# JunweiLiang/FVTA_MemexQA

Hardware: AMD Instinct MI355X
Metric: QA-pairs/sec (fwd+bwd) at B=64, 40 photos x 5 streams x 30 tok, h=512 (higher is better)
Workload: dtype bf16; 1 GPU; BASELINE.json configs[2] train step (fwd+bwd+adam), shape 'metric', dense lengths; qa_pairs_per_gpu=64, albums=1, photos=40, text_streams=5, hidden=512, global_batch=64, K=6, T=1200, JQ=30, parallelism=dp1 (QA pairs sharded, flat-gradient all-reduce)

## Files before the change

fvta_memexqa_amd/csrc/attn_fwd_shadow.hip:

```cpp
#include "attn_fwd_shared.h"

namespace fvta {

typedef unsigned u32x4s __attribute__((ext_vector_type(4)));
typedef const u32x4s __attribute__((address_space(1)))* grow16_ptr;

__global__ __launch_bounds__(256) void attn_shadow_compact_kernel(AttnShape s, AttnSaved sv, const unsigned long long* __restrict__ table,
                                                                  unsigned long long* __restrict__ rowptr) {
  const int nk = blockIdx.x, T = s.T;
  const size_t nkt = (size_t)s.N * s.K * T;
  const int cnt = sv.cnt[nk];
  for (int p = threadIdx.x; p < cnt; p += 256) {
    const int t = sv.idx[(size_t)nk * T + p];
    rowptr[(size_t)nk * T + p] = table[(size_t)nk * T + t];
    rowptr[nkt + (size_t)nk * T + p] = table[nkt + (size_t)nk * T + t];
  }
}

template <int NBH, int RMODE>
__global__ __launch_bounds__(512, 1) void attn_fwd_pair16h(AttnFwdArgs a, int G_all, const unsigned long long* __restrict__ rowptr) {
  constexpr int NKS = NBH / 2;
  constexpr int NU = NBH / 16;
  static_assert(NBH % 16 == 0, "a wave's channel blocks are dealt round-robin to the 16 row lanes");
  extern __shared__ __attribute__((aligned(16))) char s_dyn[];
  half8(*s_qhi)[2][64] = reinterpret_cast<half8(*)[2][64]>(s_dyn);
  half8(*s_qlo)[2][64] = reinterpret_cast<half8(*)[2][64]>(s_dyn + (size_t)2 * NKS * 2 * 64 * sizeof(half8));
  float* s_vec = reinterpret_cast<float*>(s_dyn + (size_t)2 * 2 * NKS * 2 * 64 * sizeof(half8));
  __shared__ float s_ct[32];
  __shared__ __attribute__((aligned(16))) float s_x[8][8 * 64];
  __shared__ float s_rt[8][16];
  __shared__ int s_kstart[65], s_kcnt[64], s_kall[64], s_flat;
  __shared__ int s_pub[8], s_done[8];

  const AttnShape& s = a.s;
  const int tid = threadIdx.x, wave = tid >> 6, lane = tid & 63;
  const int pair = wave >> 1, hv = wave & 1;
  const int l15 = lane & 15, kq = lane >> 4;
  const int T = s.T, w = s.w, JP = s.JP;
  const size_t nkt = (size_t)s.N * s.K * T;
  int wg, n, g0, G;
  if (!attn_wg_index(s.N * G_all, wg) || !attn_wg_album(a.wgtab, wg, G_all, n, g0, G)) return;
  stage_question<2 * NKS, 2, 1>(a.sv, n, w, JP, tid, s_qhi, s_qlo, s_vec, s_ct);
  const uint64_t qvalid = a.sv.qvalid[(size_t)n * 2];
  if (tid == 64) deal_streams<16>(a.sv, n, s.K, s.nsplit, 4 * G, s_kstart, s_kcnt, s_kall, &s_flat);
  if (tid < 8) {
    s_pub[tid] = 0;
    s_done[tid] = 0;
  }
  __syncthreads();
  const bool writer = hv == 0 && lane == 0;
  AttnDeal dl = deal_init<4>(s_kstart, s_kcnt, s_kall, s_flat, a, n, g0, G, pair, writer);
  deal_fill_unowned<512>(dl, tid);
  const int rounds = deal_rounds<16>(dl);
  const int pwv = wave ^ 1;

  Seg cs = {0, 0, 0, 0, 0, 0}, ns = {0, 0, 0, 0, 0, 0};
  int ctl = 0, ntl = 0;
  int t_cur = 0, t_nxt = 0;
  bool v_cur = false, v_nxt = false;
  unsigned long long p_nxt = 0;
  float m_run = -INFINITY, l_run = 0.f;
  f32x4 u[NU];
  u32x4s hb[NKS];
#pragma unroll
  for (int i = 0; i < NU; ++i) u[i] = f32x4{0.f, 0.f, 0.f, 0.f};
  const unsigned long long* myptr = rowptr + (size_t)hv * nkt;
  auto rows_of = [&](const Seg& sg, int tl, int& t, bool& v, unsigned long long& p) {
    const int lr = tl * 16 + l15;
    v = lr < sg.cnt;
    const size_t at = (size_t)sg.nk * T + max(min(lr, sg.cnt - 1), 0);
    t = a.sv.idx[at];
    p = myptr[at];
  };
  bool active = next_seg<16>(dl, cs), has_n = false;
  if (active) {
    ctl = cs.t0;
    unsigned long long p_cur;
    rows_of(cs, ctl, t_cur, v_cur, p_cur);
    const grow16_ptr rowp = (grow16_ptr)(p_cur + 16 * kq);
#pragma unroll
    for (int i = 0; i < NKS; ++i) hb[i] = rowp[4 * i];
    has_n = tile_after<16>(dl, cs, ctl, ns, ntl);
    if (!has_n) {
      ns = cs;
      ntl = ctl;
    }
    rows_of(ns, ntl, t_nxt, v_nxt, p_nxt);
  }
  const int cbase = 16 * NBH * hv;
  auto unpack = [](const u32x4s q, f32x4& lo4, f32x4& hi4) {
    lo4 = f32x4{__uint_as_float(q[0] << 16), __uint_as_float(q[0] & 0xffff0000u), __uint_as_float(q[1] << 16), __uint_as_float(q[1] & 0xffff0000u)};
    hi4 = f32x4{__uint_as_float(q[2] << 16), __uint_as_float(q[2] & 0xffff0000u), __uint_as_float(q[3] << 16), __uint_as_float(q[3] & 0xffff0000u)};
  };

#pragma unroll 2
  for (int g = 0; g < rounds; ++g) {
    const bool rvalid = v_cur;
    const int t = t_cur;
    const bool allm = cs.allm != 0;
    float xown[8];
#pragma unroll
    for (int i = 0; i < 8; ++i) xown[i] = 0.f;
    if (active && !allm) {
      f32x4 ahh[2] = {f32x4{0.f, 0.f, 0.f, 0.f}, f32x4{0.f, 0.f, 0.f, 0.f}};
      f32x4 axx[2] = {f32x4{0.f, 0.f, 0.f, 0.f}, f32x4{0.f, 0.f, 0.f, 0.f}};
      f32x4 rt4 = {0.f, 0.f, 0.f, 0.f};
#pragma unroll
      for (int ks = 0; ks < NKS; ++ks) {
        f32x4 f0, f1;
        unpack(hb[ks], f0, f1);
        const int c0 = cbase + 32 * ks + 8 * kq;
        row_term2<RMODE, 4>(rt4, f0, f1, s_vec, c0, w + c0);
        const half8 hi8 = cat_h2(__builtin_bit_cast(half2v, __builtin_amdgcn_cvt_pkrtz(f0[0], f0[1])),
                                 __builtin_bit_cast(half2v, __builtin_amdgcn_cvt_pkrtz(f0[2], f0[3])),
                                 __builtin_bit_cast(half2v, __builtin_amdgcn_cvt_pkrtz(f1[0], f1[1])),
                                 __builtin_bit_cast(half2v, __builtin_amdgcn_cvt_pkrtz(f1[2], f1[3])));
        const int kg = NKS * hv + ks;
#pragma unroll
        for (int jt = 0; jt < 2; ++jt) {
          ahh[jt] = __builtin_amdgcn_mfma_f32_16x16x32_f16(hi8, s_qhi[kg][jt][lane], ahh[jt], 0, 0, 0);
          axx[jt] = __builtin_amdgcn_mfma_f32_16x16x32_f16(hi8, s_qlo[kg][jt][lane], axx[jt], 0, 0, 0);
        }
        __builtin_amdgcn_sched_barrier(0);
      }
      float rtp = (rt4[0] + rt4[1]) + (rt4[2] + rt4[3]);
      rtp += __shfl_xor(rtp, 16, 64);
      rtp += __shfl_xor(rtp, 32, 64);
      wait_flag(&s_done[pwv], g, a.fault);
      if (kq == 0) s_rt[wave][l15] = rtp;
#pragma unroll
      for (int jt = 0; jt < 2; ++jt)
#pragma unroll
        for (int i = 0; i < 4; ++i) {
          xown[jt * 4 + i] = ahh[jt][i] + axx[jt][i] * (1.f / 2048.f);
          s_x[wave][(jt * 4 + i) * 64 + lane] = xown[jt * 4 + i];
        }
    }
    asm volatile("" ::"v"(t_nxt), "v"(p_nxt));
    asm volatile("s_waitcnt lgkmcnt(0)" ::: "memory");
    if (lane == 0) post_flag(&s_pub[wave], g + 1);
    wait_flag(&s_pub[pwv], g + 1, a.fault);
    if (active) {
      float am = rvalid ? FVTA_NEG : -INFINITY;
      if (!allm) {
        float bestv;
        int bestj;
        finish_scores([&](int jt, int i) { return xown[jt * 4 + i] + s_x[pwv][(jt * 4 + i) * 64 + lane]; },
                      [&](int i) { return s_rt[wave][4 * kq + i] + s_rt[pwv][4 * kq + i]; }, s_ct, qvalid, l15, bestv, bestj);
        am = rvalid ? (s.add_tanh ? fvta_tanh(bestv) : bestv) : -INFINITY;
        if (hv == 0 && kq == 0 && rvalid) {
          a.sv.amax[(size_t)cs.nk * T + t] = am;
          a.sv.jmax[(size_t)cs.nk * T + t] = (uint8_t)bestj;
        }
      }
      asm volatile("s_waitcnt lgkmcnt(0)" ::: "memory");
      if (lane == 0) post_flag(&s_done[wave], g + 1);
      const float pr = softmax_step(am, m_run, l_run, u);
      const grow16_ptr rowp_next = (grow16_ptr)(p_nxt + 16 * kq);
#pragma unroll
      for (int i = 0; i < NKS; ++i) {
        f32x4 va, vb;
        unpack(hb[i], va, vb);
        va *= pr;
        vb *= pr;
        hb[i] = rowp_next[4 * i];
        row16_sum4(va);
        row16_sum4(vb);
        if (((2 * i) & 15) == l15) u[(2 * i) >> 4] += va;
        if (((2 * i + 1) & 15) == l15) u[(2 * i + 1) >> 4] += vb;
      }
      if (ctl + 1 == cs.t1) {
        float* part = a.part + ((size_t)cs.nk * s.nsplit + cs.slot) * (w + 4);
#pragma unroll
        for (int i = 0; i < NU; ++i) {
          const int b = 16 * i + l15;
          *reinterpret_cast<f32x4*>(part + 4 + cbase + 32 * (b >> 1) + 8 * kq + 4 * (b & 1)) = u[i];
          u[i] = f32x4{0.f, 0.f, 0.f, 0.f};
        }
        if (writer) store_partial_head(part, m_run, l_run);
        m_run = -INFINITY;
        l_run = 0.f;
      }
      active = has_n;
      if (has_n) {
        cs = ns;
        ctl = ntl;
        t_cur = t_nxt;
        v_cur = v_nxt;
        has_n = tile_after<16>(dl, cs, ctl, ns, ntl);
        if (!has_n) {
          ns = cs;
          ntl = ctl;
        }
      }
    }
    rows_of(ns, ntl, t_nxt, v_nxt, p_nxt);
  }
}

bool shadow_covers(const AttnShape& s) { return s.JT == 1 && (s.w == 512 || s.w == 1024) && s.simi != 4; }

void launch_attn_shadow_compact(const AttnShape& s, const AttnSaved& sv, const uint64_t* table, uint64_t* rowptr, hipStream_t stream) {
  hipLaunchKernelGGL(attn_shadow_compact_kernel, dim3(s.N * s.K), dim3(256), 0, stream, s, sv,
                     reinterpret_cast<const unsigned long long*>(table), reinterpret_cast<unsigned long long*>(rowptr));
}

template <int NBH, int RMODE>
static void launch_pair16h(const AttnFwdArgs& a, int G, const unsigned long long* rowptr, hipStream_t stream) {
  const size_t lds = attn_question_lds(NBH, a.s.w);
  (void)hipFuncSetAttribute((const void*)attn_fwd_pair16h<NBH, RMODE>, hipFuncAttributeMaxDynamicSharedMemorySize, (int)lds);
  hipLaunchKernelGGL((attn_fwd_pair16h<NBH, RMODE>), attn_xcd_grid(a.s.N * G), dim3(512), lds, stream, a, G, rowptr);
}

bool launch_attn_fwd_pair16h(const AttnFwdArgs& a, int G, const uint64_t* rowptr, hipStream_t stream) {
  const AttnShape& s = a.s;
  if (!shadow_covers(s)) return false;
  const unsigned long long* rp = reinterpret_cast<const unsigned long long*>(rowptr);
  attn_with_rmode(s.simi, [&](auto rm) {
    if (s.w == 1024)
      launch_pair16h<32, decltype(rm)::value>(a, G, rp, stream);
    else
      launch_pair16h<16, decltype(rm)::value>(a, G, rp, stream);
  });
  return true;
}

}
```

Measured before the change: 5308 QA-pairs/s.

## Use MFMA selector matmul to transpose-reduce value rows in attention forward

Replaces the per-row bf16 unpack, scale-by-probability and cross-lane row16 reduction in the value accumulation with two MFMA 16x16x32 bf16 ops. The B operand is a one-hot selector matrix, so the MFMA redistributes channels across lanes, and each lane then FMAs four shuffled probabilities into its accumulator. The partial-output writeback changes to match: accumulators are reduced across lane groups with xor-shuffles before the store. This removes many DPP/shuffle reductions per tile in exchange for matrix-core issue, a changed accumulator layout, and extra shuffles at segment end.

```diff
diff --git a/fvta_memexqa_amd/csrc/attn_fwd_shadow.hip b/fvta_memexqa_amd/csrc/attn_fwd_shadow.hip
--- a/fvta_memexqa_amd/csrc/attn_fwd_shadow.hip
+++ b/fvta_memexqa_amd/csrc/attn_fwd_shadow.hip
@@ -4,6 +4,7 @@
 
 typedef unsigned u32x4s __attribute__((ext_vector_type(4)));
 typedef const u32x4s __attribute__((address_space(1)))* grow16_ptr;
+typedef __bf16 bf16x8s __attribute__((ext_vector_type(8)));
 
 __global__ __launch_bounds__(256) void attn_shadow_compact_kernel(AttnShape s, AttnSaved sv, const unsigned long long* __restrict__ table,
                                                                   unsigned long long* __restrict__ rowptr) {
@@ -20,8 +21,9 @@
 template <int NBH, int RMODE>
 __global__ __launch_bounds__(512, 1) void attn_fwd_pair16h(AttnFwdArgs a, int G_all, const unsigned long long* __restrict__ rowptr) {
   constexpr int NKS = NBH / 2;
-  constexpr int NU = NBH / 16;
-  static_assert(NBH % 16 == 0, "a wave's channel blocks are dealt round-robin to the 16 row lanes");
+  constexpr int NV = 2 * NKS;
+  constexpr int NU = NV / 4;
+  static_assert(NBH % 16 == 0, "the lane groups share a segment's channel blocks out in quarters");
   extern __shared__ __attribute__((aligned(16))) char s_dyn[];
   half8(*s_qhi)[2][64] = reinterpret_cast<half8(*)[2][64]>(s_dyn);
   half8(*s_qlo)[2][64] = reinterpret_cast<half8(*)[2][64]>(s_dyn + (size_t)2 * NKS * 2 * 64 * sizeof(half8));
@@ -88,6 +90,12 @@
     rows_of(ns, ntl, t_nxt, v_nxt, p_nxt);
   }
   const int cbase = 16 * NBH * hv;
+  u32x4s sel[2];
+#pragma unroll
+  for (int e = 0; e < 2; ++e)
+#pragma unroll
+    for (int j = 0; j < 4; ++j)
+      sel[e][j] = (kq == 2 * e + (l15 >> 3) && ((l15 & 7) >> 1) == j) ? (0x3f80u << (16 * (l15 & 1))) : 0u;
   auto unpack = [](const u32x4s q, f32x4& lo4, f32x4& hi4) {
     lo4 = f32x4{__uint_as_float(q[0] << 16), __uint_as_float(q[0] & 0xffff0000u), __uint_as_float(q[1] << 16), __uint_as_float(q[1] & 0xffff0000u)};
     hi4 = f32x4{__uint_as_float(q[2] << 16), __uint_as_float(q[2] & 0xffff0000u), __uint_as_float(q[3] << 16), __uint_as_float(q[3] & 0xffff0000u)};
@@ -156,27 +164,44 @@
       asm volatile("s_waitcnt lgkmcnt(0)" ::: "memory");
       if (lane == 0) post_flag(&s_done[wave], g + 1);
       const float pr = softmax_step(am, m_run, l_run, u);
+      float p4[4];
+#pragma unroll
+      for (int r = 0; r < 4; ++r) p4[r] = __shfl(pr, 20 * kq + r, 64);
       const grow16_ptr rowp_next = (grow16_ptr)(p_nxt + 16 * kq);
 #pragma unroll
       for (int i = 0; i < NKS; ++i) {
-        f32x4 va, vb;
-        unpack(hb[i], va, vb);
-        va *= pr;
-        vb *= pr;
+        const bf16x8s hrow = __builtin_bit_cast(bf16x8s, hb[i]);
+        f32x4 d[2];
+#pragma unroll
+        for (int e = 0; e < 2; ++e)
+          d[e] = __builtin_amdgcn_mfma_f32_16x16x32_bf16(hrow, __builtin_bit_cast(bf16x8s, sel[e]), f32x4{0.f, 0.f, 0.f, 0.f}, 0, 0, 0);
         hb[i] = rowp_next[4 * i];
-        row16_sum4(va);
-        row16_sum4(vb);
-        if (((2 * i) & 15) == l15) u[(2 * i) >> 4] += va;
-        if (((2 * i + 1) & 15) == l15) u[(2 * i + 1) >> 4] += vb;
+#pragma unroll
+        for (int e = 0; e < 2; ++e) {
+          float acc = u[i >> 1][2 * (i & 1) + e];
+#pragma unroll
+          for (int r = 0; r < 4; ++r) acc = __builtin_fmaf(p4[r], d[e][r], acc);
+          u[i >> 1][2 * (i & 1) + e] = acc;
+        }
       }
       if (ctl + 1 == cs.t1) {
         float* part = a.part + ((size_t)cs.nk * s.nsplit + cs.slot) * (w + 4);
-#pragma unroll
-        for (int i = 0; i < NU; ++i) {
-          const int b = 16 * i + l15;
-          *reinterpret_cast<f32x4*>(part + 4 + cbase + 32 * (b >> 1) + 8 * kq + 4 * (b & 1)) = u[i];
-          u[i] = f32x4{0.f, 0.f, 0.f, 0.f};
-        }
+        float h1[NV / 2], h2[NV / 4];
+#pragma unroll
+        for (int q = 0; q < NV / 2; ++q) {
+          const float lo = u[q >> 2][q & 3], hi = u[(q + NV / 2) >> 2][(q + NV / 2) & 3];
+          h1[q] = ((kq & 2) ? hi : lo) + __shfl_xor((kq & 2) ? lo : hi, 32, 64);
+        }
+#pragma unroll
+        for (int r = 0; r < NV / 4; ++r) {
+          const float lo = h1[r], hi = h1[r + NV / 4];
+          h2[r] = ((kq & 1) ? hi : lo) + __shfl_xor((kq & 1) ? lo : hi, 16, 64);
+        }
+        float* pu = part + 4 + cbase + 16 * ((NV / 2) * (kq >> 1) + (NV / 4) * (kq & 1)) + l15;
+#pragma unroll
+        for (int r = 0; r < NV / 4; ++r) pu[16 * r] = h2[r];
+#pragma unroll
+        for (int i = 0; i < NU; ++i) u[i] = f32x4{0.f, 0.f, 0.f, 0.f};
         if (writer) store_partial_head(part, m_run, l_run);
         m_run = -INFINITY;
         l_run = 0.f;
```

After: 5320 QA-pairs/s, median of 6. No clear change (+0.2%).
